# CaiLiLab/MuRaL

Hardware: AMD Instinct MI355X
Metric: predicted bases/s (SNV local=10/distal=1000, 4-class, predict) (higher is better)
Workload: dtype f32; 1 GPU; SNV default predict, synthetic 10M positions (BASELINE.json configs[1]); local_radius=10, distal_radius=1000, n_class=4, input=2-bit packed genome resident in HBM, every site's full window, weights=weights_init, torch.manual_seed(0), parallelism=dp1, collective=none

## Files before the change

mural_amd/csrc/encode.hip:

```cpp
#include <cstring>
#include <cstdlib>
#include "common.h"
#include "dense_symbol.h"

namespace mural {

static thread_local std::string g_err;

void set_error(const char* fmt, ...) {
  char buf[1024];
  va_list ap;
  va_start(ap, fmt);
  vsnprintf(buf, sizeof(buf), fmt, ap);
  va_end(ap);
  g_err = buf;
}

const char* last_error_cstr() { return g_err.c_str(); }

bool g_dev_switches = false;

const DevSwitch* dev_switch_table() {
  static const DevSwitch table[] = {
    {"MURAL_TOWER_DYNAMIC_UNITS", "A/B, bit-identical: SNV predict units through a global ticket counter instead of the fixed stride"},
    {"MURAL_SNV_DEFER_SHORT", "A/B, bit-identical: =0 runs the short-stage launches per chunk (what a one-chunk workspace does by itself)"},
    {"MURAL_LOCAL_REG", "A/B, bit-identical: =0 keeps the local MLP's weight fragments in LDS (snv_local_mlp_mfma)"},
    {"MURAL_INDEL_CHUNK", "A/B, same results: positions per pass of the INDEL layer program (256 .. 4096; default 2048)"},
    {"MURAL_TRAIN_CONV_CL", "A/B: the training step on the workgroup-tile conv kernels (conv32_cl.hip) instead of the wave-private ones"},
    {"MURAL_TRAIN_NO_FIRST_FOLD", "A/B: the first stage's last BatchNorm-backward apply as a pass of its own"},
    {"MURAL_TRAIN_NO_MID_FOLD", "A/B: the short stage's last apply as a pass of its own"},
    {"MURAL_TRAIN_NO_POOL_FOLD", "A/B: the applies in front of the pools as passes of their own"},
    {"MURAL_TRAIN_LOCAL_OPS", "A/B: the local branch of the training step as per-op launches"},
    {"MURAL_TRAIN_HEAD_OPS", "A/B: a tower's head of the training step as per-op launches"},
    {"MURAL_TRAIN_FIRST_SEPARATE", "A/B: symbol histograms / first-layer tables per tower"},
    {"MURAL_XCD_SWIZZLE", "A/B, bit-identical: =0 disables the XCD-aware workgroup index of the barrier-free INDEL kernels"},
    {"MURAL_CONVBLOCK_DIRECT", "A/B: 0 / 2 never / always the barrier-free ConvBlock"},
    {"MURAL_CONVBLOCK8_VALU", "A/B: the 8-channel ConvBlock entirely on the vector ALU"},
    {"MURAL_INDEL_ENC0", "A/B: =0 disables the persistent level-0 encoder launch"},
    {"MURAL_INDEL_ENC0_DOWN", "A/B: =0 keeps the stride-4 down-conv a launch of its own"},
    {"MURAL_INDEL_DEC0", "A/B: =0 disables the persistent level-0 decoder launch"},
    {"MURAL_INDEL_DEEP", "A/B: =0 runs the deep levels' blocks as two launches each"},
    {"MURAL_INDEL_DEEP_FRONT", "A/B: =0 keeps the fourth level's strided conv a launch of its own"},
    {"MURAL_INDEL_DENSE_SYMBOLS", "A/B: =0 keeps the dense INDEL entry on the three-launch route"},
    {"MURAL_WGRAD_MFMA", "A/B: =0 keeps the INDEL weight gradients on the LDS-tiled vector kernel"},
    {"MURAL_DEBUG_WS_GUARD", "validation: unused bytes behind every workspace region (tests poison and check them)"},
    {"MURAL_DEBUG_DROP_PART_ROW", "validation (fault injection): drop one partial row of a conv weight gradient"},
    {"MURAL_DEBUG_NO_SMALL_BATCH", "validation: calls of <= 256 sites through the throughput launches"},
    {"MURAL_DEBUG_NO_LONGWIN", "validation: long windows through the per-layer path"},
    {"MURAL_DEBUG_LOCAL_VALU", "validation: the local MLP on the vector ALU"},
    {"MURAL_DEBUG_INDEL_NO_GENOME_FRONT", "validation: the packed INDEL entry through an explicit one-hot tensor"},
    {"MURAL_DEBUG_TOWER_RUNTIME_GEOM", "validation, bit-identical: the first-stage tower instance that reads its geometry from the arguments"},
    {"MURAL_DEBUG_POLY_NARROW", "validation: the polyphase up-conv's dword stores"},
    {"MURAL_DEBUG_FIRST_SCATTER", "validation: the first layer's backward through LDS atomics"},
    {"MURAL_DEBUG_S1_ALIAS", "TIMING ONLY, wrong results: every site writes the x0 rows of site (row mod 64)"},
    {"MURAL_DEBUG_CW", "TIMING ONLY, wrong results: phases of the wave-private conv kernels switched off (bit mask)"},
    {"MURAL_DEBUG_MLP", "TIMING ONLY, wrong results: phases of the local MLP switched off"},
    {"MURAL_DEBUG_CB_STAMP_ONLY", "diagnostic: phase stamps of one workgroup only"},
    {nullptr, nullptr}};
  return table;
}

const char* dev_env(const char* name) {
  if (!g_dev_switches) return nullptr;
  for (const DevSwitch* s = dev_switch_table(); s->name; ++s)
    if (!std::strcmp(s->name, name)) return std::getenv(name);
  std::fprintf(stderr, "libmural_hip (debug flavour): %s is read but not listed in dev_switch_table\n", name);
  return nullptr;
}

int dev_int(const char* name, int dflt) {
  const char* e = dev_env(name);
  return e ? atoi(e) : dflt;
}

thread_local std::vector<size_t> g_ws_layout;

size_t ws_guard_bytes() {
  const char* e = dev_env("MURAL_DEBUG_WS_GUARD");
// ... 222 lines not shown
```

mural_amd/csrc/snv.h:

```cpp
#pragma once
#include "common.h"

namespace mural {

constexpr int SNV_C = 32;
constexpr int SNV_K = 3;
constexpr int SNV_NLAYER = 10;
constexpr int SNV_KSTEPS = 24;
constexpr int SNV_WFRAG = 2 * SNV_KSTEPS * 64;
constexpr int SNV_LUT = 125 * SNV_C;
constexpr int SNV_TAPS = 3 * N_SYM * SNV_C;
constexpr int SNV_LUTBLK = SNV_LUT + SNV_TAPS + SNV_C;
constexpr int SNV_LUT4 = 256 * SNV_C;
constexpr int SNV_MAXCLASS = 16;
constexpr int SNV_CHUNK = 131072;
constexpr int SNV_NB2MAX = 9;
constexpr int SNV_THREADS = 256;
constexpr int SNV_WAVES = SNV_THREADS / 64;
constexpr int SNV_MID_HALF = 100;

enum { L_RB1A_C1 = 0, L_RB1A_C2, L_RB1B_C1, L_RB1B_C2, L_CONV2, L_RB2A_C1, L_RB2A_C2, L_RB2B_C1, L_RB2B_C2, L_CONV3 };
enum { EX_RB1_ENTRY = 0, EX_BN_MID = 1, EX_BN_OUT = 2, EX_FC_BN = 3, EX_COUNT = 4 };

struct TowerGeom {
// ... 74 lines not shown
  const float* gamma;
  const double* acc;
  double n;
  float* dgamma;
  float* dbeta;
};
struct FirstTrainArgs {
  Stage1Tower tw;
  int Lwin, cw, wave_bytes;
  int64_t B;
  const uint8_t* sym;
  const float* lutblk;
  float* y;
  uint8_t* arg;
  const float* dy;
  float* dpart;
  int cl;
  double* stat;
  FirstFold fold;
  unsigned long long* stamps;
};
extern unsigned long long* g_first_stamps;
int first_train_grid(int64_t B);
bool first_train_supported(int C, int pk);
bool first_train_fits(int Lwin, int L2, int pk);
int launch_first_train(FirstTrainArgs a, bool bwd, hipStream_t stream);

struct SnvFwdArgs {
  TowerGeom geom[2];
  TowerDev tw[2];
  int P;
  int nbuf;
  int Lwin;
  int n_class;
  int has_local;
  int64_t n;
  const float* x0;
  int x0_cols;
  const float* local_logits;
  float* out;
  float* taps;
  int tap_stride;
  unsigned long long* stamps;
  const int32_t* status;
  int tw_first, tw_last;
  float* xlogit;
  int par;
  float* xlogit2;
  int* tile_count;
  int phase;
  float* s3[2];
  int wave;
  int* unit_counter;
  int seg_n, seg_step, seg_col0;
};

constexpr int RU_EC = 9;
constexpr int RU_EV = 5;
constexpr int RU_L = 2 * RU_EC;
constexpr int RU_SC = RU_L + 1;

struct EdgeArgs {
  TowerDev tw;
  int64_t n;
  const int64_t* pos;
  const uint8_t* strand;
  int64_t glen;
  int64_t t0[2], nb;
  int woff;
  int L1;
  int L2, L3;
  int D;
  int pk2, ps2, pp2;
  int u_lo, u_hi;
  int right_pad;
  const float* F[2];
  const float* El[2];
  const float* Er[2];
  const float* R[2];
  const float* S[2];
  float* s3;
};

constexpr int EW_P = 7;
size_t edge_wave_lds_bytes();
int launch_snv_edge_wave(const EdgeArgs& e, int* unit_counter, hipStream_t stream);

}

struct MuralSnvModel {
  MuralSnvShape shape;
  mural::SnvFwdArgs args;
  mural::SnvFwdArgs args_split[4];
  size_t lds_split[4];
  bool split;
  mural::SnvFwdArgs args_small;
  size_t lds_small;
  mural::LocalDev local;
  float* blob;
  size_t blob_floats;
  size_t lds_bytes;
  mural::Stage1Args s1;
  size_t s1_lds_bytes;
  bool s1_pair;
  bool loc_fused;
  mural::LocalMfmaDims loc_d;
  size_t loc_lds;
  bool longwin;
  bool front_only;
  bool front_mid;
  int lw_nA, lw_LA, lw_LB, lw_SB, lw_nj;
  mural::SnvFwdArgs args_lwA, args_lwB;
  size_t lds_lwA, lds_lwB;
  int64_t chunk;
};

namespace mural {
bool stage1_small_batch(int64_t n);
int launch_snv_stage1(const Stage1Args& a, bool packed, size_t lds_bytes, hipStream_t stream);
int launch_snv_local(const LocalDev& L, const int64_t* cat, int64_t n, float* out, hipStream_t stream);
int launch_snv_towers(const MuralSnvModel* m, const SnvFwdArgs& a, size_t lds_bytes, hipStream_t stream);
int profile_begin();
int profile_end(double* total_ms, int64_t* launches);
size_t plan_wave_geometry(SnvFwdArgs& a, int Lwin, int Pw, int n_class, int tower, int phase);
int launch_snv_tower_wave(const SnvFwdArgs& a, size_t lds_bytes, hipStream_t stream);
int launch_snv_tower_wave_jobs(const SnvFwdArgs* jobs, const size_t* lds_bytes, int n, hipStream_t stream);
extern unsigned long long* g_tower_stamps;
}
```

mural_amd/csrc/snv_model.hip:

```cpp
#include <algorithm>
#include <cmath>
#include <cstdio>
#include <cstdlib>
#include <cstring>
#include <vector>

#include "snv.h"
#include "snv_local_mfma.h"

namespace mural {

namespace {

const double kSymVec[15][4] = {
    {1, 0, 0, 0}, {0, 1, 0, 0}, {0, 0, 1, 0}, {0, 0, 0, 1}, {.25, .25, .25, .25},
    {.5, 0, .5, 0}, {0, .5, 0, .5}, {.5, .5, 0, 0}, {0, .5, .5, 0}, {.5, 0, 0, .5}, {0, 0, .5, .5},
    {0, 1. / 3, 1. / 3, 1. / 3}, {1. / 3, 0, 1. / 3, 1. / 3}, {1. / 3, 1. / 3, 0, 1. / 3}, {1. / 3, 1. / 3, 1. / 3, 0}};

struct Blob {
  std::vector<float> host;
  size_t alloc(size_t n) {
    size_t off = (host.size() + 63) & ~size_t(63);
    host.resize(off + n, 0.f);
    return off;
// ... 182 lines not shown
  emit(o.w1t, n1b, K1p / 16, in1, h1);
  emit(o.w2t, n2b, K2p / 16, h1, h2);
  emit(o.w3t, 1, K3p / 16, h2, nc);
  return MURAL_OK;
}

int pool_len(int L, int k, int s, int p) { return (L + 2 * p - k) / s + 1; }

size_t plan_geometry(SnvFwdArgs& a, int Lwin, int P, int n_class, int towers = 3, int phase = 0) {
  static const int pools[2][3][3] = {{{15, 15, 7}, {7, 7, 3}, {3, 3, 1}}, {{3, 3, 1}, {3, 3, 1}, {3, 3, 1}}};
  int maxcols = 0;
  for (int tw = 0; tw < 2; ++tw) {
    TowerGeom& g = a.geom[tw];
    g.L1 = tw == 0 ? Lwin : 2 * SNV_MID_HALF + 1;
    g.col0 = tw == 0 ? 0 : Lwin / 2 - SNV_MID_HALF;
    int L = g.L1;
    for (int i = 0; i < 3; ++i) {
      g.pk[i] = pools[tw][i][0];
      g.ps[i] = pools[tw][i][1];
      g.pp[i] = pools[tw][i][2];
      L = pool_len(L, g.pk[i], g.ps[i], g.pp[i]);
      if (L < 1) return 0;
      g.L[i] = L;
      g.Sc[i] = L + 1;
      g.NC[i] = 1 + P * g.Sc[i];
      g.nb[i] = (g.NC[i] + 15) / 16;
      g.dL[i] = FastDiv::make((uint32_t)L);
      g.dSc[i] = FastDiv::make((uint32_t)g.Sc[i]);
      if (!((towers >> tw) & 1)) continue;
      if ((phase == 1 && i != 0) || (phase == 2 && i == 0)) continue;
      if ((g.nb[i] + 1) / 2 > SNV_NB2MAX) return 0;
      maxcols = std::max(maxcols, 16 * g.nb[i] + 2);
    }
  }
  a.P = P;
  a.Lwin = Lwin;
  a.tw_first = (towers & 1) ? 0 : 1;
  a.tw_last = (towers & 2) ? 1 : 0;
  a.phase = phase;
  a.x0_cols = a.geom[0].L[0] + a.geom[1].L[0];
  a.nbuf = maxcols * SNV_C;
  const size_t par = (size_t)2 * (2 * EX_COUNT * SNV_C + n_class * SNV_C + SNV_MAXCLASS);
  return (size_t)2 * a.nbuf * 4 + (size_t)(2 * P * SNV_C + 3 * P * SNV_MAXCLASS) * 4 + par * 4;
}

constexpr size_t kLdsTwoPerCu = 80 * 1024;
constexpr size_t kLdsMax = 160 * 1024;

size_t align_up(size_t v, size_t a) { return (v + a - 1) / a * a; }

struct Workspace { float* local_logits; int64_t* cat; uint8_t* symbols; float* x0; float* xlogit; float* s3[2]; int* counters;
                   float *vx0A, *vx0B, *vs3A, *vs3B; };

constexpr int SNV_SUPER = 4;
int64_t super_chunk_sites(const MuralSnvModel* m) {
  const bool off = dev_int("MURAL_SNV_DEFER_SHORT", 1) == 0;
  return (m->split && !m->longwin && !off) ? SNV_SUPER * m->chunk : m->chunk;
}

size_t carve(const MuralSnvModel* m, int64_t n, bool dense, void* base, Workspace* w, bool one_chunk = false) {
  size_t off = 0;
  const size_t guard = ws_guard_bytes();
  ws_layout_reset();
  auto take = [&](size_t bytes) {
    size_t o = off;
    ws_layout_add(o, bytes);
    off = align_up(off + bytes + guard, 256);
    return o;
  };
  const size_t o_ll = take((size_t)n * m->shape.n_class * 4);
  const size_t o_cat = take((size_t)n * std::max(m->shape.local_cols, 1) * 8);
  const size_t o_sym = take(dense ? (size_t)n * m->shape.distal_len : 16);
  const size_t o_x0 = take((size_t)std::min<int64_t>(n, m->chunk) * std::max(m->args.x0_cols, 1) * SNV_C * 4);
  const int64_t s3_sites = std::min<int64_t>(n, one_chunk ? m->chunk : super_chunk_sites(m));
  const size_t o_xl = take((size_t)s3_sites * SNV_MAXCLASS * 4);
  const size_t o_s3l = take((size_t)s3_sites * std::max(m->args.geom[0].L[1], 1) * SNV_C * 4);
  const size_t o_s3m = take((size_t)s3_sites * std::max(m->args.geom[1].L[1], 1) * SNV_C * 4);
  const size_t o_cnt = take(64);
  size_t o_vxa = 0, o_vxb = 0, o_vsa = 0, o_vsb = 0;
  if (m->longwin) {
    const size_t cn = (size_t)std::min<int64_t>(n, m->chunk);
    (void)o_vxa;
    (void)o_vxb;
    o_vsa = take(cn * m->lw_nA * m->args_lwA.geom[0].L[1] * SNV_C * 4);
    o_vsb = take(cn * m->args_lwB.geom[0].L[1] * SNV_C * 4);
  }
  if (w) {
    char* b = static_cast<char*>(base);
    w->local_logits = reinterpret_cast<float*>(b + o_ll);
    w->cat = reinterpret_cast<int64_t*>(b + o_cat);
    w->symbols = reinterpret_cast<uint8_t*>(b + o_sym);
    w->x0 = reinterpret_cast<float*>(b + o_x0);
    w->xlogit = reinterpret_cast<float*>(b + o_xl);
    w->s3[0] = reinterpret_cast<float*>(b + o_s3l);
    w->s3[1] = reinterpret_cast<float*>(b + o_s3m);
    w->counters = reinterpret_cast<int*>(b + o_cnt);
    w->vx0A = reinterpret_cast<float*>(b + o_vxa);
    w->vx0B = reinterpret_cast<float*>(b + o_vxb);
    w->vs3A = reinterpret_cast<float*>(b + o_vsa);
    w->vs3B = reinterpret_cast<float*>(b + o_vsb);
  }
  return off;
}

__global__ void lw_scatter_kernel(const float* __restrict__ vs, int64_t n, int nseg, int Lp , int nj, int j_lo,
                                  int j_hi, int jl_shift, int L3, float* __restrict__ s3) {
  const int span = j_hi - j_lo;
  const int64_t total = n * span * 8;
  for (int64_t i = blockIdx.x * (int64_t)blockDim.x + threadIdx.x; i < total; i += (int64_t)gridDim.x * blockDim.x) {
    const int q = (int)(i & 7);
    const int64_t col = i >> 3;
    const int j = j_lo + (int)(col % span);
    const int64_t site = col / span;
    int k = j <= nj ? 0 : (j - 1) / nj;
    if (k > nseg - 1) k = nseg - 1;
    const int jl = j - k * nj + jl_shift;
    const float4 v = reinterpret_cast<const float4*>(vs + (((size_t)site * nseg + k) * Lp + jl) * SNV_C)[q];
    reinterpret_cast<float4*>(s3 + ((size_t)site * L3 + j) * SNV_C)[q] = v;
  }
}

void fill_tower_lengths(SnvFwdArgs& a, int Lwin) {
  static const int pools[2][3][3] = {{{15, 15, 7}, {7, 7, 3}, {3, 3, 1}}, {{3, 3, 1}, {3, 3, 1}, {3, 3, 1}}};
  for (int tw = 0; tw < 2; ++tw) {
    TowerGeom& g = a.geom[tw];
    g.L1 = tw == 0 ? Lwin : 2 * SNV_MID_HALF + 1;
    g.col0 = tw == 0 ? 0 : Lwin / 2 - SNV_MID_HALF;
// ... 208 lines not shown
    L.b2 = m->blob + loff.b2; L.w3t = m->blob + loff.w3t; L.b3 = m->blob + loff.b3;
    L.frag = m->blob + loff.frag; L.frag_floats = (int)loff.frag_floats;
    L.cols = sh.local_cols; L.emb_rows = sh.emb_rows; L.in1 = 5 * sh.local_cols; L.h1 = sh.hidden1; L.h2 = sh.hidden2;
    L.n_class = sh.n_class;
    m->loc_fused = has_towers && local_mfma_plan(L, &m->loc_d, &m->loc_lds);
  }
  *out = m;
  return MURAL_OK;
}

extern "C" void mural_snv_model_destroy(MuralSnvModel* m) {
  if (!m) return;
  if (m->blob) (void)hipFree(m->blob);
  delete m;
}

extern "C" size_t mural_snv_workspace_bytes(const MuralSnvModel* m, int64_t n, int32_t dense) {
  if (!m || n <= 0) return 256;
  return carve(m, n, dense != 0, nullptr, nullptr);
}

extern "C" size_t mural_snv_workspace_bytes_min(const MuralSnvModel* m, int64_t n, int32_t dense) {
  if (!m || n <= 0) return 256;
  return carve(m, n, dense != 0, nullptr, nullptr, true);
}

extern "C" int mural_snv_tap_layout(const MuralSnvModel* m, int32_t* o) {
  MURAL_REQUIRE(m && o, "NULL argument");
  std::memset(o, 0, 16 * sizeof(int32_t));
  o[0] = m->args.P;
  o[1] = m->args.nbuf;
  for (int i = 0; i < 3; ++i) { o[2 + i] = m->args.geom[0].L[i]; o[5 + i] = m->args.geom[1].L[i]; }
  o[8] = 13;
  o[9] = (int32_t)m->lds_bytes;
  o[10] = m->front_only ? 1 : 0;
  o[11] = (int32_t)m->chunk;
  o[12] = m->front_mid ? 1 : 0;
  return MURAL_OK;
}

extern "C" const char* mural_snv_kernel_name(void) { return "snv_tower_wave"; }

extern "C" int mural_profile_begin(void) { return mural::profile_begin(); }
extern "C" int mural_profile_end(double* total_ms, int64_t* launches) { return mural::profile_end(total_ms, launches); }

namespace mural { unsigned long long* g_tower_stamps = nullptr; }

constexpr int64_t SNV_SMALL_BATCH = 256;

static int run_towers(const MuralSnvModel* m, Stage1Args s1, SnvFwdArgs a, bool packed, int64_t n, const Workspace& w,
                      float* out, float* taps, const int32_t* status, hipStream_t stream, bool one_chunk = false, float* front_out = nullptr) {
  const int nc = m->shape.n_class;
  const bool small = taps == nullptr && n <= SNV_SMALL_BATCH && m->lds_small > 0 && !dev_env("MURAL_DEBUG_NO_SMALL_BATCH");
  const bool defer = m->split && taps == nullptr && !small && !m->longwin && super_chunk_sites(m) > m->chunk && n > m->chunk && !one_chunk;
  const int64_t super = defer ? super_chunk_sites(m) : m->chunk;
  const size_t s3l_site = (size_t)std::max(m->args.geom[0].L[1], 1) * SNV_C, s3m_site = (size_t)std::max(m->args.geom[1].L[1], 1) * SNV_C;
  for (int64_t sc0 = 0; sc0 < n; sc0 += super) {
  const int64_t sn = std::min<int64_t>(super, n - sc0);
  for (int64_t c0 = sc0; c0 < sc0 + sn; c0 += m->chunk) {
    const int64_t cn = std::min<int64_t>(m->chunk, sc0 + sn - c0);
    const int64_t rel = defer ? c0 - sc0 : 0;
    Stage1Args s = s1;
    s.n = cn;
    s.x0 = w.x0;
    s.zero = small ? reinterpret_cast<int*>(w.s3[1]) : nullptr;
    if (packed) { s.pos = s1.pos + c0; s.strand = s1.strand + c0; }
    else s.codes = s1.codes + c0 * m->shape.distal_len;
    if (int rc = launch_snv_stage1(s, packed, s.loc_on ? std::max(m->s1_lds_bytes, m->loc_lds) : m->s1_lds_bytes, stream)) return rc;
    const bool split = m->split && taps == nullptr && !small;
    if (split && dev_int("MURAL_TOWER_DYNAMIC_UNITS", 0) != 0)
      MURAL_HIP_CHECK(hipMemsetAsync(w.counters, 0, 64, stream));
    bool lw_mid_done = false;
    for (int part = 0; part < (split ? (defer ? 2 : 4) : 1); ++part) {
      if (part == 1 && lw_mid_done) continue;
      if (m->longwin && part == 0) {
        const int LpA = m->args_lwA.geom[0].L[1], LpB = m->args_lwB.geom[0].L[1], L3 = m->args.geom[0].L[1], nj = m->lw_nj;
        const int x0_cols = m->args.x0_cols;
        auto grid_of = [](int64_t items) { return dim3((unsigned)std::min<int64_t>((items + 255) / 256, 65536)); };
        SnvFwdArgs lw_jobs[3];
        size_t lw_lds[3];
        const bool lw_merge = m->args_lwA.wave && m->args_lwB.wave && m->args_split[1].wave && (!front_out || m->front_mid);
        for (int kind = 0; kind < 2; ++kind) {
          SnvFwdArgs t = kind == 0 ? m->args_lwA : m->args_lwB;
          t.n = kind == 0 ? cn * m->lw_nA : cn;
          t.x0 = w.x0;
          t.x0_cols = x0_cols;
          t.seg_n = kind == 0 ? m->lw_nA : 1;
          t.seg_step = kind == 0 ? 7 * nj : 0;
          t.seg_col0 = kind == 0 ? 0 : m->lw_SB;
          t.s3[0] = kind == 0 ? w.vs3A : w.vs3B;
          t.s3[1] = w.s3[1];
          t.xlogit = w.xlogit;
          t.local_logits = w.local_logits + c0 * nc;
          t.out = out ? out + c0 * nc : nullptr;
          t.taps = nullptr;
          t.stamps = nullptr;
          t.status = status;
          t.unit_counter = w.counters + 4 + kind;
          if (lw_merge) {
            lw_jobs[kind] = t;
            lw_lds[kind] = kind == 0 ? m->lds_lwA : m->lds_lwB;
          } else if (int rc = launch_snv_towers(m, t, kind == 0 ? m->lds_lwA : m->lds_lwB, stream)) {
            return rc;
          }
        }
        if (lw_merge) {
          SnvFwdArgs t = m->args_split[1];
          t.s3[0] = w.s3[0];
          t.s3[1] = w.s3[1];
          t.n = cn;
          t.x0 = w.x0;
          t.xlogit = w.xlogit;
          t.local_logits = w.local_logits + c0 * nc;
          t.out = out ? out + c0 * nc : nullptr;
          t.taps = nullptr;
          t.tap_stride = a.nbuf;
          t.stamps = nullptr;
          t.status = status;
          t.unit_counter = nullptr;
          lw_jobs[2] = t;
          lw_lds[2] = m->lds_split[1];
          if (int rc = launch_snv_tower_wave_jobs(lw_jobs, lw_lds, 3, stream)) return rc;
          lw_mid_done = true;
        }
        const int jA = m->lw_nA * nj + 1;
        float* s3_dst = front_out ? front_out + (size_t)c0 * L3 * SNV_C : w.s3[0];
        hipLaunchKernelGGL(lw_scatter_kernel, grid_of(cn * jA * 8), dim3(256), 0, stream, w.vs3A, cn, m->lw_nA, LpA, nj, 0, jA, 0, L3, s3_dst);
        if (L3 > jA)
          hipLaunchKernelGGL(lw_scatter_kernel, grid_of(cn * (L3 - jA) * 8), dim3(256), 0, stream, w.vs3B, cn, 1, LpB, nj, jA, L3,
                             -(m->lw_SB / 7), L3, s3_dst);
        MURAL_HIP_CHECK(hipGetLastError());
        if (front_out && !m->front_mid) break;
        continue;
      }
      if (front_out && part > 1) break;
      SnvFwdArgs t = split ? m->args_split[part] : (small ? m->args_small : a);
      t.s3[0] = w.s3[0] + (size_t)rel * s3l_site;
      t.s3[1] = w.s3[1] + (size_t)rel * s3m_site;
      t.n = cn;
      t.x0 = w.x0;
      t.xlogit = w.xlogit + (size_t)rel * SNV_MAXCLASS;
      if (small) {
        t.par = 1;
        t.xlogit2 = w.s3[0];
        t.tile_count = reinterpret_cast<int*>(w.s3[1]);
      }
      t.local_logits = w.local_logits + c0 * nc;
      t.out = out ? out + c0 * nc : nullptr;
      t.taps = c0 == 0 ? taps : nullptr;
      t.tap_stride = a.nbuf;
      t.stamps = packed ? mural::g_tower_stamps : nullptr;
      t.status = status;
      t.unit_counter = split && t.wave ? w.counters + part : nullptr;
      size_t lds = split ? m->lds_split[part] : (small ? m->lds_small : m->lds_bytes);
      if (split && !t.wave && part >= 2 && t.P > 1) {
        const int want = (int)std::max<int64_t>(1, std::min<int64_t>(t.P, (cn + 511) / 512));
        if (want < t.P) {
          SnvFwdArgs t2 = t;
          const size_t need = plan_geometry(t2, m->shape.distal_len, want, m->shape.n_class, (part & 1) ? 2 : 1, 2);
          if (need && need <= lds) {
            t = t2;
            lds = need;
          }
        }
      }
      if (int rc = launch_snv_towers(m, t, lds, stream)) return rc;
    }
  }
  if (defer) {
    for (int part = 2; part < 4; ++part) {
      SnvFwdArgs t = m->args_split[part];
      t.s3[0] = w.s3[0];
      t.s3[1] = w.s3[1];
      t.n = sn;
      t.x0 = w.x0;
      t.xlogit = w.xlogit;
      t.local_logits = w.local_logits + sc0 * nc;
      t.out = out + sc0 * nc;
      t.taps = nullptr;
      t.tap_stride = a.nbuf;
      t.stamps = packed ? mural::g_tower_stamps : nullptr;
      t.status = status;
      t.unit_counter = t.wave ? w.counters + part : nullptr;
      if (int rc = launch_snv_towers(m, t, m->lds_split[part], stream)) return rc;
    }
  }
  }
  return MURAL_OK;
}

static bool local_rides(const MuralSnvModel* m, int64_t n) { return m->shape.model_no == 2 && m->loc_fused && stage1_small_batch(n); }
static void ride_local(const MuralSnvModel* m, Stage1Args* s1, const int64_t* cat, float* logits) {
  s1->loc_on = 1;
  s1->loc = m->local;
  s1->loc_d = m->loc_d;
  s1->loc_cat = cat;
  s1->loc_out = logits;
}

static int forward_dense_impl(const MuralSnvModel* m, const int64_t* cat_x, const float* distal_x, int64_t n, float* out,
                              void* workspace, size_t ws_bytes, int32_t* status, float* taps, size_t taps_floats,
                              void* stream_, const uint8_t* symbols = nullptr) {
  MURAL_REQUIRE(m, "model handle is NULL");
  MURAL_REQUIRE(!m->front_only, "distal_radius %d: only the first conv stage of this model runs fused (mural_snv_forward_front)", (m->shape.distal_len - 1) / 2);
  MURAL_REQUIRE(n >= 0, "negative batch");
  if (n == 0) return MURAL_OK;
  hipStream_t stream = (hipStream_t)stream_;
  const MuralSnvShape& sh = m->shape;
  MURAL_REQUIRE(out, "out is NULL");
  const bool own_symbols = symbols == nullptr;
  const bool one_chunk = ws_bytes < carve(m, n, own_symbols, nullptr, nullptr);
  if (ws_bytes < carve(m, n, own_symbols, nullptr, nullptr, true) || !workspace) {
    set_error("workspace too small: need %zu bytes, got %zu", carve(m, n, own_symbols, nullptr, nullptr, true), ws_bytes);
    return MURAL_E_WORKSPACE;
  }
  Workspace w;
  carve(m, n, own_symbols, workspace, &w, one_chunk);
  if (sh.model_no == 0) {
    MURAL_REQUIRE(cat_x, "cat_x is NULL");
    return launch_snv_local(m->local, cat_x, n, out, stream);
  }
  MURAL_REQUIRE(distal_x || symbols, "distal_x is NULL");
  if (sh.model_no == 2) {
    MURAL_REQUIRE(cat_x, "cat_x is NULL");
    if (!local_rides(m, n))
      if (int rc = launch_snv_local(m->local, cat_x, n, w.local_logits, stream)) return rc;
  }
  const bool direct = stage1_small_batch(n) && !symbols;
  if (!direct && !symbols)
    if (int rc = launch_dense_to_symbols(distal_x, n, sh.distal_len, w.symbols, status, stream)) return rc;
  if (taps) MURAL_REQUIRE(!m->longwin, "the layer dump is not available for long windows (segmented first stage)");
  if (taps) MURAL_REQUIRE(taps_floats >= (size_t)13 * m->args.nbuf, "taps buffer too small (need %zu floats)", (size_t)13 * m->args.nbuf);
  Stage1Args s1 = m->s1;
  s1.codes = symbols ? symbols : w.symbols;
  if (direct) {
    s1.dense = distal_x;
    s1.status = status;
  }
  if (local_rides(m, n)) ride_local(m, &s1, cat_x, w.local_logits);
// ... 128 lines not shown
```

mural_amd/csrc/snv_tower_wave.hip:

```cpp
#include <cstdlib>
#include <cstring>
#include <type_traits>

#include "snv_tower_conv.h"

namespace mural {

template <int M>
using ModeTag = std::integral_constant<int, M>;
__host__ __device__ constexpr TowerGeom wave_tower_geom(int tw, int Lwin, int Pw) {
  constexpr int pools[2][3][3] = {{{15, 15, 7}, {7, 7, 3}, {3, 3, 1}}, {{3, 3, 1}, {3, 3, 1}, {3, 3, 1}}};
  TowerGeom g{};
  g.L1 = tw == 0 ? Lwin : 2 * SNV_MID_HALF + 1;
  g.col0 = tw == 0 ? 0 : Lwin / 2 - SNV_MID_HALF;
  int L = g.L1;
  for (int i = 0; i < 3; ++i) {
    g.pk[i] = pools[tw][i][0];
    g.ps[i] = pools[tw][i][1];
    g.pp[i] = pools[tw][i][2];
    L = (L + 2 * g.pp[i] - g.pk[i]) / g.ps[i] + 1;
    g.L[i] = L;
    if (L < 1) return g;
    g.Sc[i] = L + 1;
    g.NC[i] = 1 + Pw * g.Sc[i];
// ... 494 lines not shown
        for (int r = 3; r < n_rounds; ++r) {
          const int u = args.u_lo + 8 * r + u_l;
          if (u <= args.u_hi) {
            const f32x4 v = ok ? buf_ld4(srs, (uint32_t)u * sstep + 16u * (uint32_t)cg) : splat(__uint_as_float(0x7FC00000u));
            __builtin_amdgcn_raw_buffer_store_b128(__builtin_bit_cast(u32x4, v), drs, (uint32_t)u * 128u + 16u * (uint32_t)cg, 0, 0);
          }
        }
      }
      const int n_edge = args.L3 - n_int;
#pragma unroll 1
      for (int task = lane_o; task < Pw * n_edge * 8; task += 64) {
        const int pj = task >> 3;
        const int p = pj / n_edge, e = pj - p * n_edge;
        const int u = e < args.u_lo ? e : args.u_hi + 1 + (e - args.u_lo);
        if (row0 + p >= args.n) continue;
        const int64_t ws = wst[p];
        f32x4 m = splat(__uint_as_float(0x7FC00000u));
        if (ws >= 0) {
          const int set = (int)(ws >> 62);
          const int64_t w = ws & ((1ll << 62) - 1);
          const int jlo = u * args.ps2 - args.pp2;
          const int lo = jlo < 0 ? 0 : jlo;
          const int hi = (jlo + args.pk2 - 1) < (args.L2 - 1) ? (jlo + args.pk2 - 1) : (args.L2 - 1);
          f32x4 rv[7];
#pragma unroll
          for (int d = 0; d < 7; ++d) {
            rv[d] = splat(-INFINITY);
            const int q = lo + d;
            if (q <= hi) {
              if (q < RU_EV) rv[d] = ld4(img + lds_off(1 + p * RU_SC + q + 1, cg));
              else if (q > args.L2 - 1 - RU_EV) rv[d] = ld4(img + lds_off(1 + p * RU_SC + (q - (args.L2 - RU_L)) + 1, cg));
              else rv[d] = ld4(args.R[set] + (size_t)(w + (int64_t)args.D * q) * 32 + 4 * cg);
            }
          }
          m = max4(max4(max4(rv[0], rv[1]), max4(rv[2], rv[3])), max4(max4(rv[4], rv[5]), rv[6]));
          for (int q = lo + 7; q <= hi; ++q) {
            f32x4 v;
            if (q < RU_EV) v = ld4(img + lds_off(1 + p * RU_SC + q + 1, cg));
            else if (q > args.L2 - 1 - RU_EV) v = ld4(img + lds_off(1 + p * RU_SC + (q - (args.L2 - RU_L)) + 1, cg));
            else v = ld4(args.R[set] + (size_t)(w + (int64_t)args.D * q) * 32 + 4 * cg);
            m = max4(m, v);
          }
          m = f32x4{fmaf(pool_s.x, m.x, pool_t.x), fmaf(pool_s.y, m.y, pool_t.y), fmaf(pool_s.z, m.z, pool_t.z),
                    fmaf(pool_s.w, m.w, pool_t.w)};
        }
        st4(args.s3 + ((size_t)(row0 + p) * args.L3 + u) * 32 + 4 * cg, m);
      }
    }
    cur ^= 1;
  }
}

static bool tower_dynamic_units() { return dev_int("MURAL_TOWER_DYNAMIC_UNITS", 0) != 0; }

size_t edge_wave_lds_bytes() {
  return (size_t)(4 * SNV_C + 4 * 3 * SNV_C + SNV_WAVES * ((16 * EW_NB + 2) * SNV_C + EW_WST + TW_DUMP)) * 4;
}

int launch_snv_edge_wave(const EdgeArgs& e, int* unit_counter, hipStream_t stream) {
  const int64_t n_units = (e.n + EW_P - 1) / EW_P;
  const int64_t n_wg = (n_units + SNV_WAVES - 1) / SNV_WAVES;
  if (n_wg == 0) return MURAL_OK;
  const int grid = (int)(n_wg < 512 ? n_wg : 512);
  if (n_units < 4 * (int64_t)grid * SNV_WAVES || !tower_dynamic_units()) unit_counter = nullptr;
  static DynLdsOnce lds;
  if (int rc = lds.ensure(&snv_edge_wave)) return rc;
  hipLaunchKernelGGL(snv_edge_wave, dim3(grid), dim3(SNV_THREADS), edge_wave_lds_bytes(), stream, e, unit_counter);
  MURAL_HIP_CHECK(hipGetLastError());
  return MURAL_OK;
}

size_t plan_wave_geometry(SnvFwdArgs& a, int Lwin, int Pw, int n_class, int tower, int phase) {
  int maxcols = 0;
  for (int tw = 0; tw < 2; ++tw) {
    a.geom[tw] = wave_tower_geom(tw, Lwin, Pw);
    const TowerGeom& g = a.geom[tw];
    for (int i = 0; i < 3; ++i) {
      if (g.L[i] < 1) return 0;
      if (tw != tower) continue;
      if ((phase == 1 && i != 0) || (phase == 2 && i == 0)) continue;
      if (g.nb[i] > TW_NBW) return 0;
      if (phase == 1 && g.nb[i] != TW_NBW) return 0;
      maxcols = std::max(maxcols, 16 * g.nb[i] + 2);
    }
  }
  if (Pw > 31) return 0;
  if (phase == 2 && !(Lwin == SHIP_LWIN && Pw == (tower == 0 ? 6 : 5))) return 0;
  a.P = Pw;
  a.Lwin = Lwin;
  a.tw_first = tower;
  a.tw_last = tower;
  a.phase = phase;
  a.wave = 1;
  a.x0_cols = a.geom[0].L[0] + a.geom[1].L[0];
  a.nbuf = maxcols * SNV_C;
  const size_t par = (size_t)(2 * EX_COUNT * SNV_C + n_class * SNV_C + SNV_MAXCLASS + 4 + 6 * 3 * SNV_C);
  const size_t per_wave = (size_t)a.nbuf + (phase == 2 ? (size_t)Pw * SNV_C + 3 * (size_t)Pw * SNV_MAXCLASS : 0) + TW_DUMP;
  return (par + SNV_WAVES * per_wave) * 4;
}

int launch_snv_tower_wave_jobs(const SnvFwdArgs* jobs_in, const size_t* lds_bytes, int n, hipStream_t stream) {
  MURAL_REQUIRE(n >= 1 && n <= 3, "wave-private tower launch: %d jobs", n);
  SnvFwdJobs jobs;
  std::memset(&jobs, 0, sizeof(jobs));
  int gx = 0, ny = 0;
  size_t lds = 0;
  int64_t wg_of[3] = {0, 0, 0};
  for (int i = 0; i < n; ++i) {
    const SnvFwdArgs& a = jobs_in[i];
    MURAL_REQUIRE(a.phase == 1 && a.Lwin != SHIP_LWIN, "wave-private tower jobs: first-stage launches of the run-time-geometry instance only");
    const int64_t n_units = (a.n + a.P - 1) / a.P;
    const int64_t n_wg = (n_units + SNV_WAVES - 1) / SNV_WAVES;
    if (n_wg == 0) continue;
    jobs.j[ny] = a;
    jobs.j[ny].unit_counter = nullptr;
    wg_of[ny] = n_wg;
    lds = lds_bytes[i] > lds ? lds_bytes[i] : lds;
    ++ny;
  }
  if (ny == 0) return MURAL_OK;
  for (int i = 0; i < ny; ++i) {
    jobs.grid[i] = (int)(wg_of[i] < 512 ? wg_of[i] : 512);
    gx = jobs.grid[i] > gx ? jobs.grid[i] : gx;
  }
  static DynLdsOnce big_lds;
  if (int rc = big_lds.ensure(&snv_tower_wave_jobs<1, 9, 0>)) return rc;
  hipLaunchKernelGGL((snv_tower_wave_jobs<1, 9, 0>), dim3(gx, ny), dim3(SNV_THREADS), lds, stream, jobs);
  MURAL_HIP_CHECK(hipGetLastError());
  return MURAL_OK;
}

int launch_snv_tower_wave(const SnvFwdArgs& a_in, size_t lds_bytes, hipStream_t stream) {
  SnvFwdArgs a = a_in;
  const int64_t n_units = (a.n + a.P - 1) / a.P;
  const int64_t n_wg = (n_units + SNV_WAVES - 1) / SNV_WAVES;
  if (n_wg == 0) return MURAL_OK;
  const int resident = 512;
  const int grid = (int)(n_wg < resident ? n_wg : resident);
  if (n_units < 4 * (int64_t)grid * SNV_WAVES || !tower_dynamic_units()) a.unit_counter = nullptr;
  static DynLdsOnce big_lds;
  if (int rc = big_lds.ensure(&snv_tower_wave<1, 9, 0, 0, 1>, &snv_tower_wave<1, 9, 0, 1, 2>, &snv_tower_wave<2, 8, 4, 0, 6>,
                              &snv_tower_wave<2, 8, 3, 1, 5>, &snv_tower_wave<1, 9, 0>)) return rc;
  const int t = a.tw_first;
  const int ship_pw = a.phase == 1 ? (t == 0 ? 1 : 2) : (t == 0 ? 6 : 5);
  bool ship = a.Lwin == SHIP_LWIN && a.P == ship_pw && !(a.phase == 1 && dev_env("MURAL_DEBUG_TOWER_RUNTIME_GEOM"));
  if (ship) {
    const TowerGeom want = wave_tower_geom(t, SHIP_LWIN, ship_pw), other = wave_tower_geom(0, SHIP_LWIN, 1);
    const TowerGeom& have = a.geom[t];
    for (int i = 0; i < 3; ++i)
      ship = ship && have.L[i] == want.L[i] && have.Sc[i] == want.Sc[i] && have.NC[i] == want.NC[i] && have.nb[i] == want.nb[i] &&
             have.pk[i] == want.pk[i] && have.ps[i] == want.ps[i] && have.pp[i] == want.pp[i];
    ship = ship && a.geom[0].L[0] == other.L[0] && a.x0_cols == other.L[0] + wave_tower_geom(1, SHIP_LWIN, 1).L[0];
  }
  const dim3 gr(grid), bl(SNV_THREADS);
  if (a.phase == 1) {
    if (ship && t == 0) hipLaunchKernelGGL((snv_tower_wave<1, 9, 0, 0, 1>), gr, bl, lds_bytes, stream, a);
    else if (ship) hipLaunchKernelGGL((snv_tower_wave<1, 9, 0, 1, 2>), gr, bl, lds_bytes, stream, a);
    else hipLaunchKernelGGL((snv_tower_wave<1, 9, 0>), gr, bl, lds_bytes, stream, a);
  } else {
    if (ship && t == 0) hipLaunchKernelGGL((snv_tower_wave<2, 8, 4, 0, 6>), gr, bl, lds_bytes, stream, a);
    else if (ship) hipLaunchKernelGGL((snv_tower_wave<2, 8, 3, 1, 5>), gr, bl, lds_bytes, stream, a);
    else {
      set_error("internal: short-stage wave launch without the shipped geometry");
      return MURAL_E_INVALID;
    }
  }
  MURAL_HIP_CHECK(hipGetLastError());
  return MURAL_OK;
}

}
```

mural_amd/csrc/snv_tower_wave_body.inc:

```
  extern __shared__ __attribute__((aligned(16))) float smem[];
  const int tid = threadIdx.x;
  const int lane = tid & 63;
  const int wave = __builtin_amdgcn_readfirstlane(tid >> 6);
  const int n16 = lane & 15, kk = lane >> 4;
  constexpr bool SHIP = TWC >= 0;
  const int Pw = SHIP ? PWC : args.P;
  const int tw_i = SHIP ? TWC : args.tw_first;
  unsigned long long t_prev = args.stamps != nullptr ? __builtin_amdgcn_s_memtime() : 0ull;
  if (args.stamps != nullptr && lane == 0) {
    unsigned long long* row = args.stamps + (size_t)(1024 + 2 * SNVW_BX + (wave >> 1)) * 32;
    row[((PHASE - 1) * 2 + tw_i) * 4 + 2 * (wave & 1)] = __builtin_amdgcn_s_memrealtime();
    if (PHASE == 1 && tw_i == 0) {
      row[16 + 2 * (wave & 1)] = __builtin_amdgcn_s_getreg((31 << 11) | (0 << 6) | 4);
      row[17 + 2 * (wave & 1)] = __builtin_amdgcn_s_getreg((3 << 11) | (0 << 6) | 20);
    }
  }
  constexpr TowerGeom g_ship = wave_tower_geom(SHIP ? TWC : 0, SHIP_LWIN, SHIP ? PWC : 1);
  const TowerGeom& g_arg = args.geom[SHIP ? 0 : tw_i];
  const TowerGeom& g = SHIP ? g_ship : g_arg;
  const TowerDev& tw = args.tw[tw_i];
  const int L0_large = SHIP ? wave_tower_geom(0, SHIP_LWIN, 1).L[0] : args.geom[0].L[0];
  const int x0_cols = SHIP ? wave_tower_geom(0, SHIP_LWIN, 1).L[0] + wave_tower_geom(1, SHIP_LWIN, 1).L[0] : args.x0_cols;
  const int x0c = tw_i == 0 ? 0 : L0_large;
  const int lpar0 = 2 * EX_COUNT * SNV_C + args.n_class * SNV_C + SNV_MAXCLASS + 4;
  const int par_floats = lpar0 + 6 * 3 * SNV_C;
  float* par = smem;
  const int wave_floats = args.nbuf + (PHASE == 2 ? Pw * SNV_C + 3 * Pw * SNV_MAXCLASS : 0) + TW_DUMP;
  const uint32_t dump0 = 4u * (uint32_t)(wave_floats - TW_DUMP);
  float* img = smem + par_floats + wave * wave_floats;
  float* feat = img + args.nbuf;
  float* logit = feat + Pw * SNV_C;
  for (int i = tid; i < EX_COUNT * SNV_C; i += SNV_THREADS) {
    par[i] = tw.ex_s[i];
    par[EX_COUNT * SNV_C + i] = tw.ex_t[i];
  }
  for (int i = tid; i < args.n_class * SNV_C; i += SNV_THREADS) par[2 * EX_COUNT * SNV_C + i] = tw.fc_w[i];
  if (tid < args.n_class) par[2 * EX_COUNT * SNV_C + args.n_class * SNV_C + tid] = tw.fc_b[tid];
  {
    const int l0 = PHASE == 1 ? 0 : 4, nl = PHASE == 1 ? 4 : 6;
    for (int i = tid; i < nl * SNV_C; i += SNV_THREADS) {
      const int l = i >> 5, c = i & 31;
      par[lpar0 + (l * 3 + 0) * SNV_C + c] = tw.bias[(l0 + l) * 32 + c];
      par[lpar0 + (l * 3 + 1) * SNV_C + c] = tw.post_s[(l0 + l) * 32 + c];
      par[lpar0 + (l * 3 + 2) * SNV_C + c] = tw.post_t[(l0 + l) * 32 + c];
    }
  }
  {
    const int st0 = PHASE == 1 ? 0 : 1;
    if (lane < 8) st4(img + lds_off(0, lane), splat(0.f));
    else if (lane < 16) st4(img + lds_off(16 * g.nb[st0] + 1, lane - 8), splat(0.f));
    if (PHASE == 1) wave_zero_gaps(img, g, 0, Pw, lane);
  }
  __syncthreads();

  const int64_t n_units = (args.n + Pw - 1) / Pw;
  const bool dyn = args.unit_counter != nullptr;
  const int64_t unit_step = (int64_t)SNVW_GX * SNV_WAVES;
  int ticket = 0;
  int64_t unit0 = (int64_t)SNVW_BX * SNV_WAVES + wave;
  if (dyn) {
    if (lane == 0) ticket = atomicAdd(args.unit_counter, 1);
    unit0 = __builtin_amdgcn_readfirstlane(ticket);
    if (lane == 0) ticket = atomicAdd(args.unit_counter, 1);
  }
  char* imgb = reinterpret_cast<char*>(img);
  const int chv0 = 4 * kk, chv1 = 16 + 4 * kk;

  f32x4 xr0[TW_NBW], xr1[TW_NBW];
  float a0[SNV_KSTEPS], a1[SNV_KSTEPS];
  const int first_layer = PHASE == 1 ? 0 : 4;
  const int last_layer = PHASE == 1 ? 3 : SNV_NLAYER - 1;
  FragSrc fsrc;
  fsrc.wf = uniform_rsrc(tw.wfrag4);
  fsrc.lane16 = 16u * (uint32_t)lane;
  fsrc.layer_bytes = (uint32_t)first_layer * SNV_WFRAG * 4u;
#pragma unroll
  for (int g4 = 0; g4 < SNV_KSTEPS / 4; ++g4) load_frag4(a0, a1, fsrc, g4);
  const WaveAddr sa_a = wave_setup(g, PHASE == 1 ? 0 : 1, Pw, n16, kk, dump0);
  if (PHASE == 1) wave_request_x0(args, g, Pw, x0_cols, x0c, xr0, xr1, unit0, n_units, n16, kk);
  const bool do_head = PHASE == 2 && args.tw_last == 1 && args.tw_first == 1;
  bool tile_ready = false;
  XReq xoff;
  xoff.base = uniform_rsrc(args.x0);
  xoff.dSc = g.dSc[0];
  xoff.Sc = (uint32_t)g.Sc[0];
  xoff.L = (uint32_t)g.L[0];
  xoff.rows = (uint32_t)Pw;
  xoff.x0_cols = (uint32_t)x0_cols;
  xoff.lane_col = (uint32_t)n16;
  xoff.kk16 = 16u * (uint32_t)kk;
  xoff.on = false;

  for (int64_t unit = unit0, next_unit = 0; unit < n_units; unit = next_unit) {
    const int64_t row0 = unit * Pw;
    if (dyn) {
      next_unit = __builtin_amdgcn_readfirstlane(ticket);
      if (lane == 0) ticket = atomicAdd(args.unit_counter, 1);
    } else {
      next_unit = unit + unit_step;
    }
    if (PHASE == 1) {
      const f32x4 es0 = ld4(par + EX_RB1_ENTRY * 32 + chv0), et0 = ld4(par + (EX_COUNT + EX_RB1_ENTRY) * 32 + chv0);
      const f32x4 es1 = ld4(par + EX_RB1_ENTRY * 32 + chv1), et1 = ld4(par + (EX_COUNT + EX_RB1_ENTRY) * 32 + chv1);
#pragma unroll
      for (int b = 0; b < TW_NBW; ++b)
        if (b < (NBA > 0 ? NBA : g.nb[0])) {
          const bool v = (sa_a.vmask >> b) & 1u;
          lds_st4(imgb, v ? sa_a.wr[0] + TW_BLK * b : sa_a.dump, relu_bn_pk(xr0[b], es0, et0));
          lds_st4(imgb, v ? sa_a.wr[1] + TW_BLK * b : sa_a.dump, relu_bn_pk(xr1[b], es1, et1));
        }
    } else {
      const int Lout = g.L[1], ScO = g.Sc[1];
      const int total = Pw * Lout * 8;
      if (!tile_ready) {
        const int64_t left = args.n - row0;
        const uint32_t bytes = (uint32_t)(left < Pw ? left : Pw) * (uint32_t)Lout * 128u;
        const __amdgpu_buffer_rsrc_t rs =
            __builtin_amdgcn_make_buffer_rsrc(const_cast<float*>(args.s3[tw_i] + (size_t)row0 * Lout * 32), 0, (int)bytes, 0x00020000);
        uint32_t l16 = 16u * (uint32_t)lane;
        asm volatile("" : "+v"(l16));
#pragma unroll
        for (int u = 0; u < 2 * TW_NBW; ++u) {
          const f32x4 v = 64 * u < total ? buf_ld4(rs, l16 + 1024u * u) : splat(0.f);
          if (u < TW_NBW) xr0[u] = v; else xr1[u - TW_NBW] = v;
        }
      }
      int lane_o = lane;
      asm volatile("" : "+v"(lane_o));
#pragma unroll
      for (int u = 0; u < 2 * TW_NBW; ++u) {
        const int task = 64 * u + lane_o;
        if (task < total) {
          const uint32_t pj = (uint32_t)task >> 3;
          const uint32_t p = g.dL[1].div(pj);
          const int jo = (int)(pj - p * (uint32_t)Lout);
          st4(img + lds_off(1 + (int)p * ScO + jo + 1, task & 7), u < TW_NBW ? xr0[u] : xr1[u - TW_NBW]);
        }
      }
      wave_zero_gaps(img, g, 1, Pw, lane_o);
      if (do_head) {
        const int64_t left = args.n - row0;
        const uint32_t rows = (uint32_t)(left < Pw ? left : Pw);
        const __amdgpu_buffer_rsrc_t xl =
            __builtin_amdgcn_make_buffer_rsrc(const_cast<float*>(args.xlogit + (size_t)row0 * SNV_MAXCLASS), 0, (int)(rows * SNV_MAXCLASS * 4u), 0x00020000);
        const __amdgpu_buffer_rsrc_t ll = __builtin_amdgcn_make_buffer_rsrc(
            const_cast<float*>(args.has_local ? args.local_logits + (size_t)row0 * args.n_class : args.xlogit), 0,
            args.has_local ? (int)(rows * (uint32_t)args.n_class * 4u) : 0, 0x00020000);
        for (int t = lane_o; t < Pw * args.n_class; t += 64) {
          const int p = t / args.n_class, k = t - p * args.n_class;
          logit[p * SNV_MAXCLASS + k] = __builtin_bit_cast(float, __builtin_amdgcn_raw_buffer_load_b32(xl, 4u * (uint32_t)(p * SNV_MAXCLASS + k), 0, 0));
          logit[(2 * Pw + p) * SNV_MAXCLASS + k] = __builtin_bit_cast(float, __builtin_amdgcn_raw_buffer_load_b32(ll, 4u * (uint32_t)t, 0, 0));
        }
// ... 206 lines not shown
```

Measured before the change: 17.24 million bases/s.

## Size SNV pieces to scratch budget and add ticket-counter tail balancing

Replaces the fixed four-chunk super-chunk deferral with one piece per call, sized to what fits a 16 GiB scratch budget, so every tower part launches once per piece over many more sites. It also adds a hybrid unit schedule: each wave follows the fixed stride for most units, then pulls its last units through an atomic ticket counter to balance the tail. This is meant to cut launch count and tail imbalance across workgroups, at the cost of a much larger workspace allocation and some atomic traffic.

After: 17.25 million bases/s, median of 6. About the same (+0.1%).

```diff
diff --git a/mural_amd/csrc/encode.hip b/mural_amd/csrc/encode.hip
--- a/mural_amd/csrc/encode.hip
+++ b/mural_amd/csrc/encode.hip
@@ -23,7 +23,10 @@
 const DevSwitch* dev_switch_table() {
   static const DevSwitch table[] = {
     {"MURAL_TOWER_DYNAMIC_UNITS", "A/B, bit-identical: SNV predict units through a global ticket counter instead of the fixed stride"},
-    {"MURAL_SNV_DEFER_SHORT", "A/B, bit-identical: =0 runs the short-stage launches per chunk (what a one-chunk workspace does by itself)"},
+    {"MURAL_TOWER_TAIL_UNITS", "A/B, bit-identical: units per wave that go through the ticket counter behind the fixed stride (0: none)"},
+    {"MURAL_TOWER_RESIDENT_WG", "validation, bit-identical: workgroups of a wave-private tower launch (1 .. 512: a small call with many units per wave)"},
+    {"MURAL_SNV_DEFER_SHORT", "A/B, bit-identical: =0 runs every launch of a call per chunk (what a one-chunk workspace does by itself)"},
+    {"MURAL_SNV_SCRATCH_SITES", "validation, bit-identical: sites per piece of a call (the workspace holds one piece; default: what fits 16 GiB)"},
     {"MURAL_LOCAL_REG", "A/B, bit-identical: =0 keeps the local MLP's weight fragments in LDS (snv_local_mlp_mfma)"},
     {"MURAL_INDEL_CHUNK", "A/B, same results: positions per pass of the INDEL layer program (256 .. 4096; default 2048)"},
     {"MURAL_TRAIN_CONV_CL", "A/B: the training step on the workgroup-tile conv kernels (conv32_cl.hip) instead of the wave-private ones"},
diff --git a/mural_amd/csrc/snv.h b/mural_amd/csrc/snv.h
--- a/mural_amd/csrc/snv.h
+++ b/mural_amd/csrc/snv.h
@@ -150,6 +150,8 @@
   float* s3[2];
   int wave;
   int* unit_counter;
+  int unit_tail;
+  int64_t unit_tail0;
   int seg_n, seg_step, seg_col0;
 };
 
@@ -222,6 +224,7 @@
 int profile_end(double* total_ms, int64_t* launches);
 size_t plan_wave_geometry(SnvFwdArgs& a, int Lwin, int Pw, int n_class, int tower, int phase);
 int launch_snv_tower_wave(const SnvFwdArgs& a, size_t lds_bytes, hipStream_t stream);
+int snv_tower_ticket_mode();
 int launch_snv_tower_wave_jobs(const SnvFwdArgs* jobs, const size_t* lds_bytes, int n, hipStream_t stream);
 extern unsigned long long* g_tower_stamps;
 }
diff --git a/mural_amd/csrc/snv_model.hip b/mural_amd/csrc/snv_model.hip
--- a/mural_amd/csrc/snv_model.hip
+++ b/mural_amd/csrc/snv_model.hip
@@ -258,10 +258,15 @@
 struct Workspace { float* local_logits; int64_t* cat; uint8_t* symbols; float* x0; float* xlogit; float* s3[2]; int* counters;
                    float *vx0A, *vx0B, *vs3A, *vs3B; };
 
-constexpr int SNV_SUPER = 4;
-int64_t super_chunk_sites(const MuralSnvModel* m) {
-  const bool off = dev_int("MURAL_SNV_DEFER_SHORT", 1) == 0;
-  return (m->split && !m->longwin && !off) ? SNV_SUPER * m->chunk : m->chunk;
+constexpr size_t kScratchCapBytes = (size_t)16 << 30;
+size_t scratch_site_bytes(const MuralSnvModel* m) {
+  return ((size_t)std::max(m->args.x0_cols, 1) + std::max(m->args.geom[0].L[1], 1) + std::max(m->args.geom[1].L[1], 1)) * SNV_C * 4 +
+         (size_t)SNV_MAXCLASS * 4;
+}
+int64_t piece_sites(const MuralSnvModel* m) {
+  if (!m->split || m->longwin || dev_int("MURAL_SNV_DEFER_SHORT", 1) == 0) return m->chunk;
+  if (const int sites = dev_int("MURAL_SNV_SCRATCH_SITES", 0); sites > 0) return sites;
+  return std::max<int64_t>(m->chunk, (int64_t)(kScratchCapBytes / scratch_site_bytes(m)));
 }
 
 size_t carve(const MuralSnvModel* m, int64_t n, bool dense, void* base, Workspace* w, bool one_chunk = false) {
@@ -277,8 +282,8 @@
   const size_t o_ll = take((size_t)n * m->shape.n_class * 4);
   const size_t o_cat = take((size_t)n * std::max(m->shape.local_cols, 1) * 8);
   const size_t o_sym = take(dense ? (size_t)n * m->shape.distal_len : 16);
-  const size_t o_x0 = take((size_t)std::min<int64_t>(n, m->chunk) * std::max(m->args.x0_cols, 1) * SNV_C * 4);
-  const int64_t s3_sites = std::min<int64_t>(n, one_chunk ? m->chunk : super_chunk_sites(m));
+  const int64_t s3_sites = std::min<int64_t>(n, one_chunk ? std::min<int64_t>(m->chunk, piece_sites(m)) : piece_sites(m));
+  const size_t o_x0 = take((size_t)s3_sites * std::max(m->args.x0_cols, 1) * SNV_C * 4);
   const size_t o_xl = take((size_t)s3_sites * SNV_MAXCLASS * 4);
   const size_t o_s3l = take((size_t)s3_sites * std::max(m->args.geom[0].L[1], 1) * SNV_C * 4);
   const size_t o_s3m = take((size_t)s3_sites * std::max(m->args.geom[1].L[1], 1) * SNV_C * 4);
@@ -593,14 +598,9 @@
                       float* out, float* taps, const int32_t* status, hipStream_t stream, bool one_chunk = false, float* front_out = nullptr) {
   const int nc = m->shape.n_class;
   const bool small = taps == nullptr && n <= SNV_SMALL_BATCH && m->lds_small > 0 && !dev_env("MURAL_DEBUG_NO_SMALL_BATCH");
-  const bool defer = m->split && taps == nullptr && !small && !m->longwin && super_chunk_sites(m) > m->chunk && n > m->chunk && !one_chunk;
-  const int64_t super = defer ? super_chunk_sites(m) : m->chunk;
-  const size_t s3l_site = (size_t)std::max(m->args.geom[0].L[1], 1) * SNV_C, s3m_site = (size_t)std::max(m->args.geom[1].L[1], 1) * SNV_C;
-  for (int64_t sc0 = 0; sc0 < n; sc0 += super) {
-  const int64_t sn = std::min<int64_t>(super, n - sc0);
-  for (int64_t c0 = sc0; c0 < sc0 + sn; c0 += m->chunk) {
-    const int64_t cn = std::min<int64_t>(m->chunk, sc0 + sn - c0);
-    const int64_t rel = defer ? c0 - sc0 : 0;
+  const int64_t piece = (one_chunk || taps != nullptr) ? std::min<int64_t>(m->chunk, piece_sites(m)) : piece_sites(m);
+  for (int64_t c0 = 0; c0 < n; c0 += piece) {
+    const int64_t cn = std::min<int64_t>(piece, n - c0);
     Stage1Args s = s1;
     s.n = cn;
     s.x0 = w.x0;
@@ -609,10 +609,12 @@
     else s.codes = s1.codes + c0 * m->shape.distal_len;
     if (int rc = launch_snv_stage1(s, packed, s.loc_on ? std::max(m->s1_lds_bytes, m->loc_lds) : m->s1_lds_bytes, stream)) return rc;
     const bool split = m->split && taps == nullptr && !small;
-    if (split && dev_int("MURAL_TOWER_DYNAMIC_UNITS", 0) != 0)
+    const int tickets = split ? snv_tower_ticket_mode() : 0;
+    const bool tail_ok = tickets == 1 && !m->longwin;
+    if (tickets == 2 || tail_ok)
       MURAL_HIP_CHECK(hipMemsetAsync(w.counters, 0, 64, stream));
     bool lw_mid_done = false;
-    for (int part = 0; part < (split ? (defer ? 2 : 4) : 1); ++part) {
+    for (int part = 0; part < (split ? 4 : 1); ++part) {
       if (part == 1 && lw_mid_done) continue;
       if (m->longwin && part == 0) {
         const int LpA = m->args_lwA.geom[0].L[1], LpB = m->args_lwB.geom[0].L[1], L3 = m->args.geom[0].L[1], nj = m->lw_nj;
@@ -676,11 +678,11 @@
       }
       if (front_out && part > 1) break;
       SnvFwdArgs t = split ? m->args_split[part] : (small ? m->args_small : a);
-      t.s3[0] = w.s3[0] + (size_t)rel * s3l_site;
-      t.s3[1] = w.s3[1] + (size_t)rel * s3m_site;
+      t.s3[0] = w.s3[0];
+      t.s3[1] = w.s3[1];
       t.n = cn;
       t.x0 = w.x0;
-      t.xlogit = w.xlogit + (size_t)rel * SNV_MAXCLASS;
+      t.xlogit = w.xlogit;
       if (small) {
         t.par = 1;
         t.xlogit2 = w.s3[0];
@@ -693,6 +695,7 @@
       t.stamps = packed ? mural::g_tower_stamps : nullptr;
       t.status = status;
       t.unit_counter = split && t.wave ? w.counters + part : nullptr;
+      t.unit_tail = t.unit_counter != nullptr && tail_ok;
       size_t lds = split ? m->lds_split[part] : (small ? m->lds_small : m->lds_bytes);
       if (split && !t.wave && part >= 2 && t.P > 1) {
         const int want = (int)std::max<int64_t>(1, std::min<int64_t>(t.P, (cn + 511) / 512));
@@ -707,25 +710,6 @@
       }
       if (int rc = launch_snv_towers(m, t, lds, stream)) return rc;
     }
-  }
-  if (defer) {
-    for (int part = 2; part < 4; ++part) {
-      SnvFwdArgs t = m->args_split[part];
-      t.s3[0] = w.s3[0];
-      t.s3[1] = w.s3[1];
-      t.n = sn;
-      t.x0 = w.x0;
-      t.xlogit = w.xlogit;
-      t.local_logits = w.local_logits + sc0 * nc;
-      t.out = out + sc0 * nc;
-      t.taps = nullptr;
-      t.tap_stride = a.nbuf;
-      t.stamps = packed ? mural::g_tower_stamps : nullptr;
-      t.status = status;
-      t.unit_counter = t.wave ? w.counters + part : nullptr;
-      if (int rc = launch_snv_towers(m, t, m->lds_split[part], stream)) return rc;
-    }
-  }
   }
   return MURAL_OK;
 }
diff --git a/mural_amd/csrc/snv_tower_wave.hip b/mural_amd/csrc/snv_tower_wave.hip
--- a/mural_amd/csrc/snv_tower_wave.hip
+++ b/mural_amd/csrc/snv_tower_wave.hip
@@ -570,6 +570,9 @@
 }
 
 static bool tower_dynamic_units() { return dev_int("MURAL_TOWER_DYNAMIC_UNITS", 0) != 0; }
+constexpr int kTowerTailUnits = 16;
+static int tower_tail_units() { return std::max(0, dev_int("MURAL_TOWER_TAIL_UNITS", kTowerTailUnits)); }
+int snv_tower_ticket_mode() { return tower_dynamic_units() ? 2 : (tower_tail_units() > 0 ? 1 : 0); }
 
 size_t edge_wave_lds_bytes() {
   return (size_t)(4 * SNV_C + 4 * 3 * SNV_C + SNV_WAVES * ((16 * EW_NB + 2) * SNV_C + EW_WST + TW_DUMP)) * 4;
@@ -653,9 +656,17 @@
   const int64_t n_units = (a.n + a.P - 1) / a.P;
   const int64_t n_wg = (n_units + SNV_WAVES - 1) / SNV_WAVES;
   if (n_wg == 0) return MURAL_OK;
-  const int resident = 512;
+  const int resident = std::min(512, std::max(1, dev_int("MURAL_TOWER_RESIDENT_WG", 512)));
   const int grid = (int)(n_wg < resident ? n_wg : resident);
-  if (n_units < 4 * (int64_t)grid * SNV_WAVES || !tower_dynamic_units()) a.unit_counter = nullptr;
+  a.unit_tail0 = 0;
+  const int64_t waves = (int64_t)grid * SNV_WAVES, per_wave = n_units / waves;
+  const int mode = snv_tower_ticket_mode();
+  if (mode == 2 && n_units >= 4 * waves) {
+  } else if (mode == 1 && a.unit_tail && a.unit_counter != nullptr && per_wave >= 2 * (int64_t)tower_tail_units()) {
+    a.unit_tail0 = (per_wave - tower_tail_units()) * waves;
+  } else {
+    a.unit_counter = nullptr;
+  }
   static DynLdsOnce big_lds;
   if (int rc = big_lds.ensure(&snv_tower_wave<1, 9, 0, 0, 1>, &snv_tower_wave<1, 9, 0, 1, 2>, &snv_tower_wave<2, 8, 4, 0, 6>,
                               &snv_tower_wave<2, 8, 3, 1, 5>, &snv_tower_wave<1, 9, 0>)) return rc;
diff --git a/mural_amd/csrc/snv_tower_wave_body.inc b/mural_amd/csrc/snv_tower_wave_body.inc
--- a/mural_amd/csrc/snv_tower_wave_body.inc
+++ b/mural_amd/csrc/snv_tower_wave_body.inc
@@ -56,12 +56,15 @@
   const int64_t n_units = (args.n + Pw - 1) / Pw;
   const bool dyn = args.unit_counter != nullptr;
   const int64_t unit_step = (int64_t)SNVW_GX * SNV_WAVES;
+  const int64_t tail0 = args.unit_tail0;
   int ticket = 0;
   int64_t unit0 = (int64_t)SNVW_BX * SNV_WAVES + wave;
   if (dyn) {
     if (lane == 0) ticket = atomicAdd(args.unit_counter, 1);
-    unit0 = __builtin_amdgcn_readfirstlane(ticket);
-    if (lane == 0) ticket = atomicAdd(args.unit_counter, 1);
+    if (unit0 >= tail0) {
+      unit0 = tail0 + __builtin_amdgcn_readfirstlane(ticket);
+      if (lane == 0) ticket = atomicAdd(args.unit_counter, 1);
+    }
   }
   char* imgb = reinterpret_cast<char*>(img);
   const int chv0 = 4 * kk, chv1 = 16 + 4 * kk;
@@ -93,11 +96,10 @@
 
   for (int64_t unit = unit0, next_unit = 0; unit < n_units; unit = next_unit) {
     const int64_t row0 = unit * Pw;
-    if (dyn) {
-      next_unit = __builtin_amdgcn_readfirstlane(ticket);
+    next_unit = unit + unit_step;
+    if (dyn && next_unit >= tail0) {
+      next_unit = tail0 + __builtin_amdgcn_readfirstlane(ticket);
       if (lane == 0) ticket = atomicAdd(args.unit_counter, 1);
-    } else {
-      next_unit = unit + unit_step;
     }
     if (PHASE == 1) {
       const f32x4 es0 = ld4(par + EX_RB1_ENTRY * 32 + chv0), et0 = ld4(par + (EX_COUNT + EX_RB1_ENTRY) * 32 + chv0);
```
